# infusionsoft/elasticsearch

Measured on AMD Instinct MI355X. Metric: docs aggregated/sec (node) + achieved HBM GB/s, terms+date_histogram, 1B docs, higher is better.
Workload: dtype int64/f64; 1 GPU; north_star; request=terms(host){date_histogram(1h){stats(response_time_ms)}}, docs_total=1000000000, collect=per shard, parallelism=1 shard(s) per GPU x1

## Files before the change

### elasticsearch_amd/csrc/check/group12_check.cpp

```cpp
#include <algorithm>
#include <cstdint>
#include <cstdio>
#include <cstdlib>
#include <random>
#include <vector>

#include "../es_group12.hpp"

static int failures = 0;
#define CHECK(cond, ...)                                  \
    do {                                                  \
        if (!(cond)) {                                    \
            ++failures;                                   \
            std::fprintf(stderr, "FAIL %s:%d: ", __FILE__, __LINE__); \
            std::fprintf(stderr, __VA_ARGS__);            \
            std::fprintf(stderr, "\n");                   \
        }                                                 \
    } while (0)

static void check_block(const std::vector<uint16_t>& rank, const std::vector<uint16_t>& d, const char* what) {
    const uint32_t n = (uint32_t)rank.size();
    std::vector<uint8_t> out(g12_block_bytes());
    std::vector<uint16_t> off(kG12OffStride, 0xDEAD);
    g12_group_block(rank.data(), d.data(), n, out.data(), off.data());
    for (uint32_t r = 0; r <= kG12Groups; ++r) {
        uint32_t below = 0;
        for (uint32_t i = 0; i < n; ++i) below += g12_group(rank[i]) < r ? 1u : 0u;
        CHECK(off[r] == below, "%s: off[%u] = %u, %u docs below", what, r, off[r], below);
    }
    for (uint32_t r = kG12Offs; r < kG12OffStride; ++r) CHECK(off[r] == 0, "%s: padding offset %u", what, r);
    CHECK(off[0] == 0 && off[kG12Groups] <= kG12Block, "%s: ends", what);
    std::vector<uint16_t> back(kG12Block);
    p12_unpack(out.data(), kG12Block, back.data());
    const auto at = [&](uint32_t j) { return (uint32_t)off[j]; };
    for (uint32_t K : {1u, 2u, 5u, 10u, 64u, 65u, kG12Groups}) {
        std::vector<std::vector<uint16_t>> got(K), want(K);
        for (uint32_t i = 0; i < n; ++i)
            if (rank[i] < K) want[rank[i]].push_back((uint16_t)(d[i] & kP12Mask));
        for (uint32_t p = 0; p < kG12Block; ++p) {
            const uint32_t r = g12_rank_at(p, K, at);
            CHECK(r <= K && (r == K) == (p >= off[K]), "%s: K %u position %u rank %u", what, K, p, r);
            if (r < K) got[r].push_back(back[p]);
        }
        for (uint32_t r = 0; r < K; ++r) {
            std::sort(got[r].begin(), got[r].end());
            std::sort(want[r].begin(), want[r].end());
            CHECK(got[r] == want[r], "%s: K %u rank %u: %zu deltas for %zu docs", what, K, r, got[r].size(), want[r].size());
        }
        for (uint32_t p0 = 0; p0 < kG12Block; p0 += 8) {
            uint32_t r8[8], s8[8];
            g12_ranks8(p0, 0, K, at, r8);
            const uint32_t w = p0 & ~511u;
            uint32_t base = 0, upto = 0;
            for (uint32_t j = 1; j <= K; ++j) {
                base += off[j] <= w ? 1u : 0u;
                upto += off[j] < w + 512u ? 1u : 0u;
            }
            g12_ranks8(p0, base, upto, at, s8);
            for (uint32_t i = 0; i < 8; ++i) {
                const uint32_t want = g12_rank_at(p0 + i, K, at);
                CHECK(r8[i] == want && s8[i] == want, "%s: K %u ranks8 at %u: %u / %u, want %u", what, K, p0 + i, r8[i], s8[i], want);
            }
        }
    }
}

int main() {
    std::mt19937 rng(20240713u);
    const auto deltas = [&](uint32_t n) {
        std::vector<uint16_t> d(n);
        for (uint16_t& x : d) x = (uint16_t)(rng() & kP12Mask);
        return d;
    };
    int blocks = 0;
    for (uint32_t n : {0u, 1u, 7u, 8u, 9u, 8191u, 8192u}) {
        for (int kind = 0; kind < 4; ++kind) {
            std::vector<uint16_t> rank(n);
            for (uint16_t& r : rank) {
                const uint32_t u = rng();
                r = kind == 0   ? (uint16_t)(u % 5)
                    : kind == 1 ? (uint16_t)std::min<uint32_t>(999, (uint32_t)(1000.0 / (1 + u % 1000)) - 1)
                    : kind == 2 ? (uint16_t)(u % 300)
                                : (u % 7 == 0 ? (uint16_t)kG12Missing : (uint16_t)(u % 200));
            }
            char what[64];
            std::snprintf(what, sizeof what, "n %u kind %d", n, kind);
            check_block(rank, deltas(n), what);
            ++blocks;
        }
    }
    {
        std::vector<uint16_t> rank(kG12Block, 0);
        check_block(rank, deltas(kG12Block), "all rank 0");
        std::fill(rank.begin(), rank.end(), (uint16_t)kG12Missing);
        check_block(rank, deltas(kG12Block), "all missing");
        std::fill(rank.begin(), rank.end(), (uint16_t)kG12Groups);
        check_block(rank, deltas(kG12Block), "all rank 128");
        for (uint32_t i = 0; i < kG12Block; ++i) rank[i] = i < 3 ? (uint16_t)(i == 2 ? 4 : 0) : i < 6 ? (uint16_t)(i == 3 ? 1 : 7) : (uint16_t)9;
        check_block(rank, deltas(kG12Block), "short runs, empty ranks");
        blocks += 4;
    }
    CHECK(g12_prefix_bytes(0) == 0 && g12_prefix_bytes(1) == 12 && g12_prefix_bytes(8) == 12 && g12_prefix_bytes(9) == 24 &&
              g12_prefix_bytes(kG12Block) == g12_block_bytes() && g12_block_bytes() == 12288,
          "prefix bytes");
    CHECK(kG12OffBytes == 260 && kG12OffBytes % 4 == 0, "offset stride");
    if (failures) {
        std::fprintf(stderr, "group12_check: %d failures\n", failures);
        return 1;
    }
    std::printf("group12_check ok: %d blocks, every position's rank for K = 1 2 5 10 64 65 128\n", blocks);
    return 0;
}
```

### elasticsearch_amd/csrc/es_group12.hpp

```cpp
#pragma once
#include "es_pack12.hpp"

constexpr uint32_t kG12Block = 8192;
constexpr uint32_t kG12Groups = 128;
constexpr uint32_t kG12Offs = kG12Groups + 1;
constexpr uint32_t kG12OffStride = (kG12Offs + 1u) & ~1u;
constexpr uint32_t kG12OffBytes = kG12OffStride * 2;
constexpr uint32_t kG12Missing = 0xFFFFu;

ES_P12_HD uint32_t g12_group(uint32_t rank) { return rank < kG12Groups ? rank : kG12Groups; }
ES_P12_HD uint64_t g12_ceil8(uint64_t n) { return (n + (kP12Group - 1)) & ~(uint64_t)(kP12Group - 1); }
ES_P12_HD size_t g12_block_bytes() { return p12_bytes(kG12Block); }
ES_P12_HD size_t g12_data_bytes(size_t n_blocks) { return n_blocks * g12_block_bytes(); }
ES_P12_HD size_t g12_off_bytes(size_t n_blocks) { return n_blocks * kG12OffBytes; }
ES_P12_HD size_t g12_prefix_bytes(uint64_t n) { return p12_bytes((size_t)g12_ceil8(n)); }

template <class OffAt>
ES_P12_HD uint32_t g12_rank_at(uint32_t p, uint32_t K, OffAt off) {
    uint32_t r = 0;
    for (uint32_t j = 1; j <= K; ++j) r += off(j) <= p ? 1u : 0u;
    return r;
}
template <class OffAt>
ES_P12_HD void g12_ranks8(uint32_t p0, uint32_t base, uint32_t upto, OffAt off, uint32_t (&r)[8]) {
    for (int i = 0; i < 8; ++i) r[i] = base;
    for (uint32_t j = base + 1; j <= upto; ++j) {
        const uint32_t o = off(j);
        for (int i = 0; i < 8; ++i) r[i] += o <= p0 + (uint32_t)i ? 1u : 0u;
    }
}

inline void g12_group_block(const uint16_t* rank, const uint16_t* d, uint32_t n, uint8_t* out, uint16_t* off) {
    uint32_t count[kG12Offs] = {};
    for (uint32_t i = 0; i < kG12Block; ++i) ++count[i < n ? g12_group(rank[i]) : kG12Groups];
    uint32_t cursor[kG12Offs], acc = 0;
    for (uint32_t g = 0; g < kG12Offs; ++g) {
        off[g] = (uint16_t)acc;
        cursor[g] = acc;
        acc += count[g];
    }
    for (uint32_t g = kG12Offs; g < kG12OffStride; ++g) off[g] = 0;
    uint16_t staged[kG12Block];
    for (uint32_t i = 0; i < kG12Block; ++i) {
        const uint32_t g = i < n ? g12_group(rank[i]) : kG12Groups;
        staged[cursor[g]++] = i < n ? (uint16_t)(d[i] & kP12Mask) : (uint16_t)0;
    }
    p12_pack(staged, kG12Block, out);
}
```

### elasticsearch_amd/csrc/esgpu_ranked_grouped.hip

```cpp
#include "es_group12.hpp"
#include "esgpu_ranked_cells.hpp"

namespace esgpu {

#ifndef ESGPU_RG_WAVES
#define ESGPU_RG_WAVES 6
#endif
constexpr uint32_t kRgPass = kRkWG * kP12Group;
static_assert(kG12Block == kBlockDocs && kBlockDocs == 2 * kRgPass, "a g12 block is a zone block: two passes of a workgroup");
static_assert(kG12Groups == 2 * 64, "a block's offsets off[1..K] are two registers of a wave");

typedef const uint32_t __attribute__((address_space(4))) rg_word_c;

struct rg_buf {
    u32x3_t v[kBlockDocs / kRgPass];
    uint32_t o0, o1;
};

__device__ __forceinline__ u32x3_t rg_load(const uint8_t* g12, uint32_t blk, uint32_t p0) {
    return __builtin_nontemporal_load(
        reinterpret_cast<const u32x3_a4_t*>(g12 + (size_t)blk * g12_block_bytes() + (p0 / kP12Group) * (kP12Words * 4)));
}

template <int MET, bool READ = true>
__device__ __forceinline__ void rg_emit(uint32_t r, uint32_t K, uint32_t cnt, uint32_t sum, uint32_t mn, uint32_t mx,
                                        uint32_t rowm, uint32_t dpk, uint32_t onehi) {
    if (r < K) {
        const uint32_t ca = rowm + 8u * r;
        atomicAdd(lds_ptr<unsigned long long>(ca + dpk), join64(sum, cnt * onehi));
        if constexpr (MET >= 2) {
            if constexpr (READ) {
                const u32x2_t m = *lds_ptr<u32x2_t>(ca);
                if (mn < m.x) atomicMin(lds_ptr<uint32_t>(ca), mn);
                if (mx > m.y) atomicMax(lds_ptr<uint32_t>(ca + 4u), mx);
            } else {
                atomicMin(lds_ptr<uint32_t>(ca), mn);
                atomicMax(lds_ptr<uint32_t>(ca + 4u), mx);
            }
        }
    }
}

template <int MET>
__device__ __forceinline__ void rg_group8(u32x3_t v, uint32_t p0, uint32_t n, uint32_t K, uint32_t base, uint32_t upto,
                                          uint32_t o0, uint32_t o1, uint32_t rowm, uint32_t dpk, uint32_t onehi) {
    if (base >= K) return;
    const uint32_t w[3] = {v.x, v.y, v.z};
    uint32_t d[8];
    if (upto == base) {
        p12_unpack8(w, d);
        const uint32_t sum = ((d[0] + d[1]) + (d[2] + d[3])) + ((d[4] + d[5]) + (d[6] + d[7]));
        const uint32_t mn = min(min(min(d[0], d[1]), min(d[2], d[3])), min(min(d[4], d[5]), min(d[6], d[7])));
        const uint32_t mx = max(max(max(d[0], d[1]), max(d[2], d[3])), max(max(d[4], d[5]), max(d[6], d[7])));
        rg_emit<MET>(base, K, 8u, sum, mn, mx, rowm, dpk, onehi);
    } else if (p0 < n) {
        p12_unpack8(w, d);
        uint32_t r[8];
        g12_ranks8(p0, base, upto, [&](uint32_t j) {
            return (uint32_t)(j <= 64 ? __builtin_amdgcn_readlane((int)o0, (int)(j - 1)) : __builtin_amdgcn_readlane((int)o1, (int)(j - 65)));
        }, r);
        uint32_t cur = r[0], cnt = 1, sum = d[0], mn = d[0], mx = d[0];
#pragma unroll
        for (int i = 1; i < 8; ++i) {
            if (r[i] != cur) {
                rg_emit<MET, false>(cur, K, cnt, sum, mn, mx, rowm, dpk, onehi);
                cur = r[i];
                cnt = 0; sum = 0; mn = ~0u; mx = 0;
            }
            ++cnt;
            sum += d[i];
            mn = min(mn, d[i]);
            mx = max(mx, d[i]);
        }
        rg_emit<MET>(cur, K, cnt, sum, mn, mx, rowm, dpk, onehi);
    }
}

template <int MET>
__global__ __launch_bounds__(kRkWG, ESGPU_RG_WAVES) void ranked_grouped_kernel(RankedParams P) {
    extern __shared__ __attribute__((aligned(16))) unsigned char smem[];
    const uint32_t K = P.K, W = P.W, C = K * W;
    const uint32_t ncp = max(P.ncopies, 1u);
    const uint32_t CS = P.cstride;
    const rk_cells cells = rk_carve<MET>(smem, C, CS, ncp);
    unsigned long long* const pk = cells.pk;
    uint32_t* const mm = cells.mm;
    const uint32_t coff = cells.coff;

    const uint32_t b_begin = blockIdx.x * P.blocks_per_wg;
    const uint32_t b_end = min(b_begin + P.blocks_per_wg, P.n_blocks);
    if (b_begin >= b_end) return;

    const uint32_t sh = P.pk_shift;
    const uint32_t onehi = 1u << (sh - 32);
    const uint32_t cell0 = MET >= 2 ? lds_addr(mm) : lds_addr(pk + coff);
    const uint32_t dpk = MET >= 2 ? lds_addr(pk + coff) - lds_addr(mm) : 0u;

    uint32_t win0 = 0;
    bool win_set = false, dirty = false;
    auto flush = [&]() { rk_flush<MET>(pk, mm, C, K, CS, ncp, sh, win0); };
    auto slide_to = [&](uint32_t k0) {
        if (dirty) flush();
        dirty = false;
        win0 = k0;
        win_set = true;
    };

    const zkey_pair_c* const zk = zkey_view(P.zkey);
    rg_word_c* const offw = (rg_word_c*)P.g12_off;
    const uint8_t* const g12 = (const uint8_t*)P.g12;
    const uint32_t lane = threadIdx.x & 63u, tid8 = threadIdx.x * kP12Group;
    const uint32_t wave0 = __builtin_amdgcn_readfirstlane(tid8 & ~(64u * kP12Group - 1u));
    const uint32_t last = b_end - 1;
    auto zload = [&](uint32_t b) -> i64x2_t { return zk[__builtin_amdgcn_readfirstlane(min(b, last))]; };
    auto nload = [&](uint32_t b) -> uint32_t {
        const uint32_t i = __builtin_amdgcn_readfirstlane(min(b, last)) * kG12OffStride + K;
        const uint32_t w = offw[i >> 1];
        return (i & 1u) ? w >> 16 : w & 0xFFFFu;
    };
    auto prefetch = [&](rg_buf& B, uint32_t blk, uint32_t n) {
        if (n > 0) {
#pragma unroll
            for (uint32_t q = 0; q < kBlockDocs / kRgPass; ++q)
                if (q * kRgPass + tid8 < n) B.v[q] = rg_load(g12, blk, q * kRgPass + tid8);
            const uint16_t* const o = P.g12_off + (size_t)blk * kG12OffStride + 1;
            if (lane < K) B.o0 = o[lane];
            if (lane + 64u < K) B.o1 = o[lane + 64u];
        }
    };
    auto block = [&](const rg_buf& B, uint32_t blk, i64x2_t z, uint32_t n) {
        const int64_t kmn = z.x, kmx = z.y;
        const bool any = kmn <= kmx && kmx >= 0 && kmn < (int64_t)P.H;
        if (any) {
            const bool fits = kmx - kmn < (int64_t)W;
            if (!win_set || (fits && (kmn < (int64_t)win0 || kmx >= (int64_t)win0 + (int64_t)W)))
                slide_to((uint32_t)min(max(kmn, (int64_t)0), (int64_t)P.H - 1));
        }
        const bool fast = kmn == kmx && (uint64_t)kmn < (uint64_t)P.H;
        if (!fast && any) {
            const auto& Q = *rk_again();
#pragma unroll 1
            for (uint32_t q = 0; q < kBlockDocs / (4u * kRkWG); ++q) {
                const uint32_t doc0 = blk * kBlockDocs + (q * kRkWG + threadIdx.x) * 4u;
                rk_r4<2> r = {0xFFFFFFFFu, 0xFFFFFFFFu};
                uint32_t m0 = 0, m1 = 0;
                if (doc0 < Q.n_docs) {
                    const u32x2_t rr = load8((const uint16_t*)Q.rank + doc0), mv = load8((const uint16_t*)Q.mv + doc0);
                    r = {rr.x, rr.y};
                    m0 = mv.x;
                    m1 = mv.y;
                }
                rk_slow_quad<MET, 2, 16>(doc0, r, m0, m1, kmn, kmx, K, win0, win_set ? W : 0u, pk, mm, coff, sh);
            }
        }
        dirty = dirty || any;
        if (fast && n > 0) {
            const uint32_t rowm = cell0 + 8u * (((uint32_t)kmn - win0) * K);
            auto span = [&](uint32_t w0, uint32_t& base, uint32_t& upto) {
                base = (uint32_t)__popcll(__ballot(B.o0 <= w0));
                upto = (uint32_t)__popcll(__ballot(B.o0 < w0 + 64u * kP12Group));
                if (K > 64u) {
                    base += (uint32_t)__popcll(__ballot(B.o1 <= w0));
                    upto += (uint32_t)__popcll(__ballot(B.o1 < w0 + 64u * kP12Group));
                }
            };
#pragma unroll
            for (uint32_t q = 0; q < kBlockDocs / kRgPass; ++q) {
                if (q * kRgPass < n) {
                    uint32_t base, upto;
                    span(q * kRgPass + wave0, base, upto);
                    rg_group8<MET>(B.v[q], q * kRgPass + tid8, n, K, base, upto, B.o0, B.o1, rowm, dpk, onehi);
                }
            }
        }
    };

    i64x2_t za = zload(b_begin), zb = zload(b_begin + 1);
    uint32_t na = nload(b_begin), nb = nload(b_begin + 1);
    rg_buf A = {{{0, 0, 0}, {0, 0, 0}}, kG12Missing, kG12Missing}, B = A;
    prefetch(A, b_begin, na);
    rk_pin();
    if (b_begin + 1 < b_end) prefetch(B, b_begin + 1, nb);
    rk_pin();
#pragma unroll 1
    for (uint32_t cb = b_begin; cb < b_end; cb += 2) {
        const i64x2_t za2 = zload(cb + 2), zb2 = zload(cb + 3);
        const uint32_t na2 = nload(cb + 2), nb2 = nload(cb + 3);
        block(A, cb, za, na);
        if (cb + 2 < b_end) prefetch(A, cb + 2, na2);
        rk_pin();
        if (cb + 1 < b_end) block(B, cb + 1, zb, nb);
        if (cb + 3 < b_end) prefetch(B, cb + 3, nb2);
        rk_pin();
        za = za2; zb = zb2;
        na = na2; nb = nb2;
    }
    if (dirty) flush();
}

template <typename F>
static auto with_rg(int met, F&& f) {
    return met >= 2 ? f(ranked_grouped_kernel<2>) : f(ranked_grouped_kernel<1>);
}
void launch_ranked_grouped(const RankedParams& p, int met, uint32_t grid, size_t lds, hipStream_t st) {
    with_rg(met, [&](auto* k) { hipLaunchKernelGGL(k, dim3(grid), dim3(kRkWG), lds, st, p); return 0; });
}
int ranked_grouped_occupancy(int met, size_t lds) {
    int n = 0;
    const hipError_t e = with_rg(met, [&](auto* k) { return hipOccupancyMaxActiveBlocksPerMultiprocessor(&n, k, kRkWG, lds); });
    return e == hipSuccess ? n : 1;
}

}
```

Measured before the change: 3218 billion docs/s.

## Pipeline ranked-grouped kernel over half-block units with four-deep prefetch slots

Replaces the two-block double buffer with a four-slot software pipeline over half-block units, skipping the second pass of blocks whose docs fit in one pass. Zone keys and per-block doc counts are loaded once per 64-block chunk into wave lanes and read with readlane, instead of scalar loads per block. Loads past a block's prefix are clamped to group 0 so tail passes stay in bounds, and a host check covers that clamping. The aim is deeper memory-level parallelism and less per-block scalar overhead, at the cost of more registers for four in-flight slots and more complex control flow.

```diff
diff --git a/elasticsearch_amd/csrc/check/group12_check.cpp b/elasticsearch_amd/csrc/check/group12_check.cpp
--- a/elasticsearch_amd/csrc/check/group12_check.cpp
+++ b/elasticsearch_amd/csrc/check/group12_check.cpp
@@ -104,6 +104,26 @@
               g12_prefix_bytes(kG12Block) == g12_block_bytes() && g12_block_bytes() == 12288,
           "prefix bytes");
     CHECK(kG12OffBytes == 260 && kG12OffBytes % 4 == 0, "offset stride");
+    {
+        std::vector<uint8_t> data(g12_block_bytes(), 1);
+        uint64_t own = 0, clamped = 0, sum = 0;
+        for (uint32_t n = 0; n <= kG12Block; ++n) {
+            for (uint32_t p0 = 0; p0 < kG12Block; p0 += kP12Group) {
+                const uint32_t g = g12_load_group(p0, n);
+                const size_t byte = (size_t)g * (kP12Words * 4);
+                const bool is_own = g == p0 / kP12Group && (uint64_t)g * kP12Group < g12_ceil8(n);
+                CHECK(is_own || g == 0, "load group: n %u p0 %u -> group %u", n, p0, g);
+                CHECK(is_own == (p0 < n) || (g == 0 && p0 == 0), "load group: n %u p0 %u own %d", n, p0, (int)is_own);
+                CHECK(byte + kP12Words * 4 <= g12_block_bytes() && byte + kP12Words * 4 <= std::max<size_t>(g12_prefix_bytes(n), kP12Words * 4),
+                      "load group: n %u p0 %u reads bytes [%zu, +12)", n, p0, byte);
+                for (uint32_t i = 0; i < kP12Words * 4; ++i) sum += data[byte + i];
+                ++(is_own ? own : clamped);
+            }
+        }
+        CHECK(sum == (own + clamped) * kP12Words * 4, "load group: bytes read");
+        std::printf("group12_check: load group over n = 0..%u: %llu own, %llu clamped to group 0\n", kG12Block, (unsigned long long)own,
+                    (unsigned long long)clamped);
+    }
     if (failures) {
         std::fprintf(stderr, "group12_check: %d failures\n", failures);
         return 1;
diff --git a/elasticsearch_amd/csrc/es_group12.hpp b/elasticsearch_amd/csrc/es_group12.hpp
--- a/elasticsearch_amd/csrc/es_group12.hpp
+++ b/elasticsearch_amd/csrc/es_group12.hpp
@@ -14,6 +14,7 @@
 ES_P12_HD size_t g12_data_bytes(size_t n_blocks) { return n_blocks * g12_block_bytes(); }
 ES_P12_HD size_t g12_off_bytes(size_t n_blocks) { return n_blocks * kG12OffBytes; }
 ES_P12_HD size_t g12_prefix_bytes(uint64_t n) { return p12_bytes((size_t)g12_ceil8(n)); }
+ES_P12_HD uint32_t g12_load_group(uint32_t p0, uint32_t n) { return p0 < n ? p0 / kP12Group : 0u; }
 
 template <class OffAt>
 ES_P12_HD uint32_t g12_rank_at(uint32_t p, uint32_t K, OffAt off) {
diff --git a/elasticsearch_amd/csrc/esgpu_ranked_grouped.hip b/elasticsearch_amd/csrc/esgpu_ranked_grouped.hip
--- a/elasticsearch_amd/csrc/esgpu_ranked_grouped.hip
+++ b/elasticsearch_amd/csrc/esgpu_ranked_grouped.hip
@@ -10,16 +10,20 @@
 static_assert(kG12Block == kBlockDocs && kBlockDocs == 2 * kRgPass, "a g12 block is a zone block: two passes of a workgroup");
 static_assert(kG12Groups == 2 * 64, "a block's offsets off[1..K] are two registers of a wave");
 
-typedef const uint32_t __attribute__((address_space(4))) rg_word_c;
-
-struct rg_buf {
-    u32x3_t v[kBlockDocs / kRgPass];
+constexpr uint32_t kRgOther = 0xFFFFFFFFu;
+constexpr uint32_t kRgChunk = 64;
+
+struct rg_slot {
+    uint32_t u;
+    uint32_t n;
+    uint32_t key;
+    u32x3_t v;
     uint32_t o0, o1;
 };
 
-__device__ __forceinline__ u32x3_t rg_load(const uint8_t* g12, uint32_t blk, uint32_t p0) {
+__device__ __forceinline__ u32x3_t rg_load(const uint8_t* g12, uint32_t blk, uint32_t p0, uint32_t n) {
     return __builtin_nontemporal_load(
-        reinterpret_cast<const u32x3_a4_t*>(g12 + (size_t)blk * g12_block_bytes() + (p0 / kP12Group) * (kP12Words * 4)));
+        reinterpret_cast<const u32x3_a4_t*>(g12 + (size_t)blk * g12_block_bytes() + g12_load_group(p0, n) * (kP12Words * 4)));
 }
 
 template <int MET, bool READ = true>
@@ -107,93 +111,104 @@
     };
 
     const zkey_pair_c* const zk = zkey_view(P.zkey);
-    rg_word_c* const offw = (rg_word_c*)P.g12_off;
     const uint8_t* const g12 = (const uint8_t*)P.g12;
     const uint32_t lane = threadIdx.x & 63u, tid8 = threadIdx.x * kP12Group;
     const uint32_t wave0 = __builtin_amdgcn_readfirstlane(tid8 & ~(64u * kP12Group - 1u));
-    const uint32_t last = b_end - 1;
-    auto zload = [&](uint32_t b) -> i64x2_t { return zk[__builtin_amdgcn_readfirstlane(min(b, last))]; };
-    auto nload = [&](uint32_t b) -> uint32_t {
-        const uint32_t i = __builtin_amdgcn_readfirstlane(min(b, last)) * kG12OffStride + K;
-        const uint32_t w = offw[i >> 1];
-        return (i & 1u) ? w >> 16 : w & 0xFFFFu;
+    uint32_t c0 = b_begin, last = b_begin, cu = 0, nv = 0, kv = 0;
+    auto fill = [&](rg_slot& S) {
+        const uint32_t blk = min(cu >> 1, last), q = cu & 1u;
+        const uint32_t n = (cu >> 1) > last ? 0u : (uint32_t)__builtin_amdgcn_readlane((int)nv, (int)(blk - c0));
+        S.u = cu;
+        S.n = n;
+        S.key = (uint32_t)__builtin_amdgcn_readlane((int)kv, (int)(blk - c0));
+        S.v = rg_load(g12, blk, q * kRgPass + tid8, n);
+        const uint16_t* const o = P.g12_off + (size_t)blk * kG12OffStride + 1;
+        S.o0 = o[min(lane, K - 1u)];
+        S.o1 = o[min(lane + 64u, K - 1u)];
+        cu = q == 0 && n > kRgPass ? cu + 1u : (cu | 1u) + 1u;
     };
-    auto prefetch = [&](rg_buf& B, uint32_t blk, uint32_t n) {
-        if (n > 0) {
-#pragma unroll
-            for (uint32_t q = 0; q < kBlockDocs / kRgPass; ++q)
-                if (q * kRgPass + tid8 < n) B.v[q] = rg_load(g12, blk, q * kRgPass + tid8);
-            const uint16_t* const o = P.g12_off + (size_t)blk * kG12OffStride + 1;
-            if (lane < K) B.o0 = o[lane];
-            if (lane + 64u < K) B.o1 = o[lane + 64u];
+    auto unit = [&](const rg_slot& S) {
+        const uint32_t blk = S.u >> 1, q = S.u & 1u, n = S.n, key = S.key;
+        if (blk > last) return;
+        const bool fast = key != kRgOther;
+        if (q == 0) {
+            int64_t kmn = key, kmx = key;
+            if (!fast) {
+                const i64x2_t z = zk[__builtin_amdgcn_readfirstlane(blk)];
+                kmn = z.x;
+                kmx = z.y;
+            }
+            const bool any = kmn <= kmx && kmx >= 0 && kmn < (int64_t)P.H;
+            if (any) {
+                const bool fits = kmx - kmn < (int64_t)W;
+                if (!win_set || (fits && (kmn < (int64_t)win0 || kmx >= (int64_t)win0 + (int64_t)W)))
+                    slide_to((uint32_t)min(max(kmn, (int64_t)0), (int64_t)P.H - 1));
+            }
+            dirty = dirty || any;
+            if (!fast && any) {
+                const auto& Q = *rk_again();
+#pragma unroll 1
+                for (uint32_t i = 0; i < kBlockDocs / (4u * kRkWG); ++i) {
+                    const uint32_t doc0 = blk * kBlockDocs + (i * kRkWG + threadIdx.x) * 4u;
+                    rk_r4<2> r = {0xFFFFFFFFu, 0xFFFFFFFFu};
+                    uint32_t m0 = 0, m1 = 0;
+                    if (doc0 < Q.n_docs) {
+                        const u32x2_t rr = load8((const uint16_t*)Q.rank + doc0), mv = load8((const uint16_t*)Q.mv + doc0);
+                        r = {rr.x, rr.y};
+                        m0 = mv.x;
+                        m1 = mv.y;
+                    }
+                    rk_slow_quad<MET, 2, 16>(doc0, r, m0, m1, kmn, kmx, K, win0, win_set ? W : 0u, pk, mm, coff, sh);
+                }
+                rk_drain();
+            }
+        }
+        if (fast && q * kRgPass < n) {
+            const uint32_t rowm = cell0 + 8u * ((key - win0) * K);
+            const uint32_t o0 = lane < K ? S.o0 : kG12Missing, o1 = lane + 64u < K ? S.o1 : kG12Missing;
+            const uint32_t w0 = q * kRgPass + wave0;
+            uint32_t base = (uint32_t)__popcll(__ballot(o0 <= w0));
+            uint32_t upto = (uint32_t)__popcll(__ballot(o0 < w0 + 64u * kP12Group));
+            if (K > 64u) {
+                base += (uint32_t)__popcll(__ballot(o1 <= w0));
+                upto += (uint32_t)__popcll(__ballot(o1 < w0 + 64u * kP12Group));
+            }
+            rg_group8<MET>(S.v, q * kRgPass + tid8, n, K, base, upto, S.o0, S.o1, rowm, dpk, onehi);
         }
     };
-    auto block = [&](const rg_buf& B, uint32_t blk, i64x2_t z, uint32_t n) {
-        const int64_t kmn = z.x, kmx = z.y;
-        const bool any = kmn <= kmx && kmx >= 0 && kmn < (int64_t)P.H;
-        if (any) {
-            const bool fits = kmx - kmn < (int64_t)W;
-            if (!win_set || (fits && (kmn < (int64_t)win0 || kmx >= (int64_t)win0 + (int64_t)W)))
-                slide_to((uint32_t)min(max(kmn, (int64_t)0), (int64_t)P.H - 1));
-        }
-        const bool fast = kmn == kmx && (uint64_t)kmn < (uint64_t)P.H;
-        if (!fast && any) {
-            const auto& Q = *rk_again();
-#pragma unroll 1
-            for (uint32_t q = 0; q < kBlockDocs / (4u * kRkWG); ++q) {
-                const uint32_t doc0 = blk * kBlockDocs + (q * kRkWG + threadIdx.x) * 4u;
-                rk_r4<2> r = {0xFFFFFFFFu, 0xFFFFFFFFu};
-                uint32_t m0 = 0, m1 = 0;
-                if (doc0 < Q.n_docs) {
-                    const u32x2_t rr = load8((const uint16_t*)Q.rank + doc0), mv = load8((const uint16_t*)Q.mv + doc0);
-                    r = {rr.x, rr.y};
-                    m0 = mv.x;
-                    m1 = mv.y;
-                }
-                rk_slow_quad<MET, 2, 16>(doc0, r, m0, m1, kmn, kmx, K, win0, win_set ? W : 0u, pk, mm, coff, sh);
-            }
-        }
-        dirty = dirty || any;
-        if (fast && n > 0) {
-            const uint32_t rowm = cell0 + 8u * (((uint32_t)kmn - win0) * K);
-            auto span = [&](uint32_t w0, uint32_t& base, uint32_t& upto) {
-                base = (uint32_t)__popcll(__ballot(B.o0 <= w0));
-                upto = (uint32_t)__popcll(__ballot(B.o0 < w0 + 64u * kP12Group));
-                if (K > 64u) {
-                    base += (uint32_t)__popcll(__ballot(B.o1 <= w0));
-                    upto += (uint32_t)__popcll(__ballot(B.o1 < w0 + 64u * kP12Group));
-                }
-            };
-#pragma unroll
-            for (uint32_t q = 0; q < kBlockDocs / kRgPass; ++q) {
-                if (q * kRgPass < n) {
-                    uint32_t base, upto;
-                    span(q * kRgPass + wave0, base, upto);
-                    rg_group8<MET>(B.v[q], q * kRgPass + tid8, n, K, base, upto, B.o0, B.o1, rowm, dpk, onehi);
-                }
-            }
-        }
-    };
-
-    i64x2_t za = zload(b_begin), zb = zload(b_begin + 1);
-    uint32_t na = nload(b_begin), nb = nload(b_begin + 1);
-    rg_buf A = {{{0, 0, 0}, {0, 0, 0}}, kG12Missing, kG12Missing}, B = A;
-    prefetch(A, b_begin, na);
-    rk_pin();
-    if (b_begin + 1 < b_end) prefetch(B, b_begin + 1, nb);
-    rk_pin();
-#pragma unroll 1
-    for (uint32_t cb = b_begin; cb < b_end; cb += 2) {
-        const i64x2_t za2 = zload(cb + 2), zb2 = zload(cb + 3);
-        const uint32_t na2 = nload(cb + 2), nb2 = nload(cb + 3);
-        block(A, cb, za, na);
-        if (cb + 2 < b_end) prefetch(A, cb + 2, na2);
-        rk_pin();
-        if (cb + 1 < b_end) block(B, cb + 1, zb, nb);
-        if (cb + 3 < b_end) prefetch(B, cb + 3, nb2);
-        rk_pin();
-        za = za2; zb = zb2;
-        na = na2; nb = nb2;
+
+    for (; c0 < b_end; c0 += kRgChunk) {
+        last = min(c0 + kRgChunk, b_end) - 1u;
+        {
+            const uint32_t bl = min(c0 + lane, last);
+            const i64x2_t z = *reinterpret_cast<const i64x2_t*>(P.zkey + 2u * (size_t)bl);
+            kv = z.x == z.y && (uint64_t)z.x < (uint64_t)P.H ? (uint32_t)z.x : kRgOther;
+            nv = P.g12_off[(size_t)bl * kG12OffStride + K];
+        }
+        cu = 2u * c0;
+        rg_slot S0, S1, S2, S3;
+        fill(S0);
+        rk_pin();
+        fill(S1);
+        rk_pin();
+        fill(S2);
+        rk_pin();
+        fill(S3);
+        rk_pin();
+        do {
+            unit(S0);
+            fill(S0);
+            rk_pin();
+            unit(S1);
+            fill(S1);
+            rk_pin();
+            unit(S2);
+            fill(S2);
+            rk_pin();
+            unit(S3);
+            fill(S3);
+            rk_pin();
+        } while ((S0.u >> 1) <= last);
     }
     if (dirty) flush();
 }
```

Measured after the change: 3627 billion docs/s, median of 6. +12.7%, better.
